# ProjectZKM/Ziren

Measured on AMD Instinct MI355X. Metric: shard-proofs/sec, higher is better.
Workload: dtype u32

## Files before the change

### include/zkm_hip.h

```cpp
#ifndef ZKM_HIP_H
#define ZKM_HIP_H

#include <stddef.h>
#include <stdint.h>

#ifdef __cplusplus
extern "C" {
#endif

#define ZKM_DIGEST_ELEMS 8
#define ZKM_EXT_DEGREE 4
#define ZKM_PERM_WIDTH 16
#define ZKM_KOALABEAR_P 0x7f000001u

typedef struct zkm_ctx zkm_ctx;
typedef struct zkm_matrix zkm_matrix;
typedef struct zkm_pcs_data zkm_pcs_data;
typedef struct zkm_pk zkm_pk;
typedef struct zkm_main_data zkm_main_data;

typedef struct {
  uint32_t log_blowup;
  uint32_t num_queries;
  uint32_t proof_of_work_bits;
// ... 44 lines not shown
const char* zkm_last_error(void);
const char* zkm_build_info(void);

int zkm_ctx_create(int device, zkm_ctx** out);
void zkm_ctx_destroy(zkm_ctx* ctx);
int zkm_ctx_synchronize(zkm_ctx* ctx);
int zkm_ctx_trim(zkm_ctx* ctx);
int zkm_ctx_set_memory_limit(zkm_ctx* ctx, size_t bytes);
size_t zkm_ctx_memory_held(zkm_ctx* ctx);
int zkm_ctx_last_timings(zkm_ctx* ctx, const char** names, float* ms, int cap);
int zkm_ctx_kernel_timings(zkm_ctx* ctx, const char** names, float* ms, uint32_t* calls, double* bytes, int cap);
void zkm_ctx_set_kernel_timing(zkm_ctx* ctx, int mode);
void zkm_ctx_set_kernel_timing_only(zkm_ctx* ctx, const char* name);
void zkm_ctx_set_lde_overlap(zkm_ctx* ctx, int on);
void zkm_ctx_set_rows_up_front(zkm_ctx* ctx, int on);
void zkm_ctx_set_host_wait(zkm_ctx* ctx, int blocking);
int zkm_ctx_register_quotient_kernel(zkm_ctx* ctx, const uint32_t* program, uint32_t program_len,
                                     const void* code_object, size_t code_object_len);

int zkm_ctx_register_perm_kernel(zkm_ctx* ctx, const uint32_t* lookups, uint32_t lookups_len, uint32_t log_quotient_degree,
                                 const void* code_object, size_t code_object_len);

void* zkm_host_alloc(zkm_ctx* ctx, size_t bytes);
void zkm_host_free(zkm_ctx* ctx, void* p);
int zkm_matrix_upload(zkm_ctx* ctx, const uint32_t* host_row_major, size_t height, size_t width,
                      zkm_matrix** out);
int zkm_matrix_upload_async(zkm_ctx* ctx, const uint32_t* host_row_major, size_t height, size_t width,
                            zkm_matrix** out);
int zkm_matrix_wait(zkm_ctx* ctx, const zkm_matrix* m);
int zkm_events_upload_async(zkm_ctx* ctx, const void* host_events, size_t bytes, void** device_events_out);
// ... 332 lines not shown
```

### integration/zkm-hip/src/ffi.rs

```rust
#![allow(non_camel_case_types, non_snake_case, dead_code)]
use core::ffi::{c_char, c_int, c_void};

pub const ZKM_DIGEST_ELEMS: u32 = 8;
pub const ZKM_EXT_DEGREE: u32 = 4;
pub const ZKM_PERM_WIDTH: u32 = 16;
pub const ZKM_KOALABEAR_P: u32 = 0x7f000001;
pub const ZKM_KECCAK_SPONGE_WIDTH: u32 = 3531;
pub const ZKM_SHA_EXTEND_WIDTH: u32 = 176;
pub const ZKM_SHA_COMPRESS_WIDTH: u32 = 262;
pub const ZKM_ED_ADD_WIDTH: u32 = 1861;
pub const ZKM_ED_DECOMPRESS_WIDTH: u32 = 1566;
pub const ZKM_GLOBAL_WIDTH: u32 = 99;

#[repr(C)] pub struct ZkmCtx { _private: [u8; 0] }
#[repr(C)] pub struct ZkmMatrix { _private: [u8; 0] }
#[repr(C)] pub struct ZkmPcsData { _private: [u8; 0] }
#[repr(C)] pub struct ZkmPk { _private: [u8; 0] }
#[repr(C)] pub struct ZkmMainData { _private: [u8; 0] }
#[repr(C)] pub struct ZkmByteLookups { _private: [u8; 0] }

#[repr(C)]
#[derive(Clone, Copy, Debug)]
pub struct ZkmFriConfig {
    pub log_blowup: u32,
// ... 412 lines not shown
extern "C" {
    pub fn zkm_last_error() -> *const c_char;
    pub fn zkm_build_info() -> *const c_char;
    pub fn zkm_ctx_create(device: c_int, out: *mut *mut ZkmCtx) -> c_int;
    pub fn zkm_ctx_destroy(ctx: *mut ZkmCtx);
    pub fn zkm_ctx_synchronize(ctx: *mut ZkmCtx) -> c_int;
    pub fn zkm_ctx_trim(ctx: *mut ZkmCtx) -> c_int;
    pub fn zkm_ctx_set_memory_limit(ctx: *mut ZkmCtx, bytes: usize) -> c_int;
    pub fn zkm_ctx_memory_held(ctx: *mut ZkmCtx) -> usize;
    pub fn zkm_ctx_last_timings(ctx: *mut ZkmCtx, names: *mut *const c_char, ms: *mut f32, cap: c_int) -> c_int;
    pub fn zkm_ctx_kernel_timings(ctx: *mut ZkmCtx, names: *mut *const c_char, ms: *mut f32, calls: *mut u32, bytes: *mut f64, cap: c_int) -> c_int;
    pub fn zkm_ctx_set_kernel_timing(ctx: *mut ZkmCtx, mode: c_int);
    pub fn zkm_ctx_set_kernel_timing_only(ctx: *mut ZkmCtx, name: *const c_char);
    pub fn zkm_ctx_set_lde_overlap(ctx: *mut ZkmCtx, on: c_int);
    pub fn zkm_ctx_set_rows_up_front(ctx: *mut ZkmCtx, on: c_int);
    pub fn zkm_ctx_set_host_wait(ctx: *mut ZkmCtx, blocking: c_int);
    pub fn zkm_ctx_register_quotient_kernel(ctx: *mut ZkmCtx, program: *const u32, program_len: u32, code_object: *const c_void, code_object_len: usize) -> c_int;
    pub fn zkm_ctx_register_perm_kernel(ctx: *mut ZkmCtx, lookups: *const u32, lookups_len: u32, log_quotient_degree: u32, code_object: *const c_void, code_object_len: usize) -> c_int;
    pub fn zkm_host_alloc(ctx: *mut ZkmCtx, bytes: usize) -> *mut c_void;
    pub fn zkm_host_free(ctx: *mut ZkmCtx, p: *mut c_void);
    pub fn zkm_matrix_upload(ctx: *mut ZkmCtx, host_row_major: *const u32, height: usize, width: usize, out: *mut *mut ZkmMatrix) -> c_int;
    pub fn zkm_matrix_upload_async(ctx: *mut ZkmCtx, host_row_major: *const u32, height: usize, width: usize, out: *mut *mut ZkmMatrix) -> c_int;
    pub fn zkm_matrix_wait(ctx: *mut ZkmCtx, m: *const ZkmMatrix) -> c_int;
    pub fn zkm_events_upload_async(ctx: *mut ZkmCtx, host_events: *const c_void, bytes: usize, device_events_out: *mut *mut c_void) -> c_int;
    pub fn zkm_events_free(ctx: *mut ZkmCtx, device_events: *mut c_void);
    pub fn zkm_matrix_download(ctx: *mut ZkmCtx, m: *const ZkmMatrix, host_row_major: *mut u32) -> c_int;
    pub fn zkm_matrix_height(m: *const ZkmMatrix) -> usize;
    pub fn zkm_matrix_width(m: *const ZkmMatrix) -> usize;
    pub fn zkm_matrix_free(ctx: *mut ZkmCtx, m: *mut ZkmMatrix);
    pub fn zkm_pcs_commit(ctx: *mut ZkmCtx, n_mats: usize, mats: *const *const ZkmMatrix, domain_shifts: *const u32, log_blowup: u32, root_out: *mut u32, out: *mut *mut ZkmPcsData) -> c_int;
// ... 84 lines not shown
```

### ziren_amd/csrc/host_ctx.hpp

```cpp
#pragma once
static thread_local std::string g_err;

#define HIP_CHECK(expr)                                                                          \
  do {                                                                                           \
    hipError_t _e = (expr);                                                                      \
    if (_e != hipSuccess)                                                                        \
      throw std::runtime_error(std::string(#expr) + ": " + hipGetErrorString(_e) + " (" + __FILE__ + ":" + \
                               std::to_string(__LINE__) + ")");                                  \
  } while (0)
#define LAUNCH_CHECK() HIP_CHECK(hipGetLastError())
#define KLAUNCH(ctx, name, bytes, kernel, grid, block, lds, ...)                                        \
  do {                                                                                                   \
    (ctx)->flush_staged();                                                                               \
    if ((ctx)->kbegin(name, (double)(bytes))) {                                                          \
       \
      hipExtLaunchKernelGGL(kernel, grid, block, lds, (ctx)->cur, (ctx)->krecs.back().start,             \
                            (ctx)->krecs.back().stop, 0, __VA_ARGS__);                                   \
    } else {                                                                                             \
      hipLaunchKernelGGL(kernel, grid, block, lds, (ctx)->cur, __VA_ARGS__);                             \
    }                                                                                                    \
    LAUNCH_CHECK();                                                                                      \
  } while (0)

static inline int log2_strict(size_t n) {
// ... 96 lines not shown
  std::mutex mu;
  std::multimap<size_t, void*> free_list;
  std::map<void*, size_t> live;
  std::map<int, uint32_t*> tw_fwd, tw_inv;
  std::vector<std::pair<std::string, hipEvent_t>> marks;
  std::vector<hipEvent_t> event_pool;
  std::vector<std::string> timing_names;
  std::vector<float> timing_ms;
  struct KRec { const char* name; double bytes; hipEvent_t start, stop; };
  struct KStat { double ms = 0, bytes = 0; uint32_t calls = 0; };
  std::vector<KRec> krecs;
  std::map<std::string, KStat> kstats;
  int kernel_timing = 2;
  bool lde_overlap = !(getenv("ZKM_LDE_OVERLAP") && atoi(getenv("ZKM_LDE_OVERLAP")) == 0);
  bool rows_up_front = !(getenv("ZKM_ROWS_UP_FRONT") && atoi(getenv("ZKM_ROWS_UP_FRONT")) == 0);
  bool root_poll = !(getenv("ZKM_ROOT_POLL") && atoi(getenv("ZKM_ROOT_POLL")) == 0);
  int root_spin_before_yield = getenv("ZKM_ROOT_SPIN") ? atoi(getenv("ZKM_ROOT_SPIN")) : 4096;
  int root_sleep_ns = getenv("ZKM_ROOT_SLEEP_NS") ? atoi(getenv("ZKM_ROOT_SLEEP_NS")) : 0;
  bool host_wait_blocking = getenv("ZKM_HOST_WAIT") && !strcmp(getenv("ZKM_HOST_WAIT"), "blocking");
  int wait_sleep_ns = getenv("ZKM_WAIT_SLEEP_NS") ? atoi(getenv("ZKM_WAIT_SLEEP_NS")) : 20000;
  struct TimerSlack {
    long saved = -1;
    void tighten() {
      if (saved >= 0) return;
      saved = prctl(PR_GET_TIMERSLACK, 0, 0, 0, 0);
      if (saved >= 0) prctl(PR_SET_TIMERSLACK, 1000UL, 0, 0, 0);
    }
    ~TimerSlack() { if (saved >= 0) prctl(PR_SET_TIMERSLACK, (unsigned long)saved, 0, 0, 0); }
  };
  static void sleep_ns(long ns, TimerSlack& slack) {
// ... 363 lines not shown
```

### ziren_amd/csrc/host_open.hpp

```cpp
#pragma once
static E4 host_pow2k(E4 a, int k) { return kb::epow2k(a, k); }

struct Writer {
  uint32_t* dst;
  size_t cap, n = 0;
  Writer(uint32_t* d, size_t c) : dst(d), cap(d ? c : 0) {}
  void u(uint32_t v) { if (n < cap) dst[n] = v; n++; }
  void words(const uint32_t* p, size_t cnt) {
    if (n < cap) memcpy(dst + n, p, std::min(cnt, cap - n) * 4);
    n += cnt;
  }
  void ext(const E4& e) { words(e.c, 4); }
  size_t size() const { return n; }
};

struct RoundMat {
  const uint32_t* evals; size_t n; size_t width; uint32_t shift;
  const zkm_matrix* lde;
  int n_points;
  std::vector<E4> y[2];
  size_t col0 = 0;
};
struct Round { const zkm_pcs_data* data; std::vector<RoundMat> mats; };

static const uint32_t SEPTIC_X[7] = {637514027, 1595065213, 1998064738, 72333738, 1211544370, 822986770, 1518535784};
static const uint32_t SEPTIC_Y[7] = {1604177449, 90440090, 259343427, 140470264, 1162099742, 941559812, 1064053343};

struct ChipMeta {
  const zkm_chip_desc* desc;
  int log_n;
  size_t n;
  int n_lookups, n_sends, perm_ext_w, max_values;
};

static ChipMeta chip_meta(const zkm_chip_desc* d, size_t n, size_t n_public_values) {
  ChipMeta m;
  m.desc = d; m.n = n; m.log_n = log2_strict(n);
  m.n_lookups = m.n_sends = m.max_values = 0;
  const std::string who = std::string(" (chip ") + (d->name ? d->name : "?") + ")";
  if (d->log_quotient_degree > 3) throw std::runtime_error("log_quotient_degree > 3 unsupported" + who);
  if (d->lookups_len) {
    const uint32_t* w = d->lookups;
    const size_t len = d->lookups_len;
    size_t pos = 0;
    auto need = [&](size_t k) { if (pos + k > len) throw std::runtime_error("lookup blob truncated" + who); };
    need(2);
    uint32_t ns = w[pos++], nr = w[pos++];
    if ((uint64_t)ns + nr > 4096) throw std::runtime_error("too many lookups" + who);
// ... 15 lines not shown
          if ((cw >> 31) ? col >= d->main_width : col >= d->prep_width) throw std::runtime_error("lookup column out of range" + who);
          if (weight >= kb::P) throw std::runtime_error("lookup weight not a field element" + who);
        }
      }
    }
    if (pos != len) throw std::runtime_error("lookup blob length mismatch" + who);
  }
  int batch = 1 << d->log_quotient_degree;
  m.perm_ext_w = m.n_lookups ? (m.n_lookups + batch - 1) / batch + 1 : 0;
  if (d->program_len) {
    if (d->program_len < 4 || d->program_len != 4 + 2 * (size_t)d->program[0]) throw std::runtime_error("program blob length mismatch" + who);
    if (d->program[2] != d->num_constraints) throw std::runtime_error("program constraint count mismatch" + who);
    const uint32_t ne = std::max<uint32_t>(d->program[1], 1), nb = std::max<uint32_t>(d->program[3], 1);
    if (ne > 256 || nb > 256) throw std::runtime_error("program register count out of range" + who);
    size_t asserts = 0;
    for (uint32_t k = 0; k < d->program[0]; k++) {
      uint32_t w0 = d->program[4 + 2 * k], imm = d->program[5 + 2 * k];
      uint32_t op = w0 & 0xff, dst = (w0 >> 8) & 0xff, ra = (w0 >> 16) & 0xff, rb = w0 >> 24;
      bool ok = true;
      switch (op) {
        case ZKM_OP_LD_MAIN: ok = dst < nb && ra < 2 && imm < d->main_width; break;
        case ZKM_OP_LD_PREP: ok = dst < nb && ra < 2 && imm < d->prep_width; break;
        case ZKM_OP_LD_PERM: ok = dst < ne && ra < 2 && imm < (uint32_t)m.perm_ext_w; break;
        case ZKM_OP_LD_CONST: ok = dst < nb && imm < kb::P; break;
        case ZKM_OP_LD_PV: ok = dst < nb && imm < n_public_values; break;
        case ZKM_OP_LD_CHALLENGE: ok = dst < ne && imm < 2; break;
        case ZKM_OP_LD_LOCAL_SUM: ok = dst < ne; break;
        case ZKM_OP_LD_GLOBAL_SUM: ok = dst < nb && imm < 14; break;
        case ZKM_OP_LD_IS_FIRST: case ZKM_OP_LD_IS_LAST: case ZKM_OP_LD_IS_TRANS: ok = dst < nb; break;
        case ZKM_OP_ADD_B: case ZKM_OP_SUB_B: case ZKM_OP_MUL_B: ok = dst < nb && ra < nb && rb < nb; break;
        case ZKM_OP_NEG_B: ok = dst < nb && ra < nb; break;
        case ZKM_OP_ADD_E: case ZKM_OP_SUB_E: case ZKM_OP_MUL_E: ok = dst < ne && ra < ne && rb < ne; break;
        case ZKM_OP_NEG_E: ok = dst < ne && ra < ne; break;
        case ZKM_OP_ADD_EB: case ZKM_OP_SUB_EB: case ZKM_OP_MUL_EB: ok = dst < ne && ra < ne && rb < nb; break;
        case ZKM_OP_ASSERT_B: ok = ra < nb; asserts++; break;
        case ZKM_OP_ASSERT_E: ok = ra < ne; asserts++; break;
        default: ok = false;
      }
      if (!ok) throw std::runtime_error("invalid instruction " + std::to_string(k) + " in constraint program" + who);
    }
    if (asserts != d->num_constraints) throw std::runtime_error("program asserts do not match num_constraints" + who);
  } else if (d->num_constraints) {
    throw std::runtime_error("num_constraints > 0 but no program" + who);
  }
  return m;
}

template <typename Alloc>
static void launch_permutation_trace(zkm_ctx* ctx, const ChipMeta& c, const uint32_t* d_blob, const uint32_t* trace, const uint32_t* prep, const E4& alpha,
                                     const E4* d_beta_powers, zkm_matrix& pt, Alloc&& salloc, std::vector<stark::ScanJob>& scans) {
  const double pbytes = 4.0 * c.n * (c.desc->main_width + c.desc->prep_width + pt.w);
  auto fit = c.desc->lookups_len ? ctx->perm_fns.find(perm_key(c.desc->lookups, c.desc->lookups_len, c.desc->log_quotient_degree)) : ctx->perm_fns.end();
  if (fit != ctx->perm_fns.end()) {
    stark::PermArgs a;
    a.main = trace; a.prep = prep; a.n = c.n; a.alpha = alpha; a.beta_pows = d_beta_powers; a.perm = pt.d;
    size_t arg_size = sizeof(a);
// ... 156 lines not shown
  for (size_t i = 0; i < nc; i++) {
    for (int e = 0; e < 4; e++) local_sums[i].c[e] = h_sums[18 * i + e];
    if (chips[i].desc->commit_scope_global) {
      for (int k = 0; k < 14; k++) global_sums[i][k] = h_sums[18 * i + 4 + k];
    } else {
      for (int k = 0; k < 7; k++) { global_sums[i][k] = kb::to_monty(SEPTIC_X[k]); global_sums[i][7 + k] = kb::to_monty(SEPTIC_Y[k]); }
    }
  }
  chal::observe_slice(ch, perm_data->root, 8);
  for (size_t i = 0; i < nc; i++) {
    chal::observe_ext(ch, local_sums[i]);
    chal::observe_slice(ch, global_sums[i].data(), 14);
  }
  }

  void quotient_phase() {
  E4 alpha = chal::sample_ext(ch);
  std::vector<std::function<void()>> launches;
  for (size_t i = 0; i < nc; i++) {
    const ChipMeta& c = chips[i];
    const zkm_chip_desc* d = c.desc;
    int lqd = d->log_quotient_degree;
    int lq = c.log_n + lqd;
    size_t Q = (size_t)1 << lq;
    size_t nchunks = (size_t)1 << lqd;
    uint32_t* qbuf = ctx->alloc_n<uint32_t>(Q * 4);
    scratch.push_back(qbuf);
    size_t C = d->num_constraints;
    std::vector<E4> ap(std::max<size_t>(C, 1));
    E4 p = kb::eone();
    for (size_t k = 0; k < C; k++) { ap[C - 1 - k] = p; p = kb::emul(p, alpha); }
    E4* d_ap = (E4*)ctx->upload_staged(ap.data(), ap.size() * sizeof(E4), &scratch);
    uint32_t consts[32] = {0};
    for (int k = 0; k < 14; k++) consts[k] = global_sums[i][k];
    uint32_t w_q = kb::two_adic_generator(lq);
    uint32_t s_pow_n = kb::pow(kb::GEN, (uint64_t)c.n);
    uint32_t wr = kb::two_adic_generator(lqd), wp = kb::ONE;
    for (size_t k = 0; k < nchunks; k++) {
      consts[16 + k] = kb::sub(kb::mul(s_pow_n, wp), kb::ONE);
      consts[24 + k] = kb::inv(consts[16 + k]);
      wp = kb::mul(wp, wr);
    }
// ... 11 lines not shown
    a.log_n = c.log_n; a.lqd = lqd;
    a.alpha_pows = d_ap; a.public_values = d_pv;
    a.perm_alpha = perm_ch[0]; a.perm_beta = perm_ch[1];
    a.local_sum = local_sums[i];
    a.consts = d_consts;
    a.w_q = w_q; a.g_inv = kb::inv(kb::two_adic_generator(c.log_n));
    a.out = qbuf;
    a.selectors = ctx->selectors(c.log_n, lqd, w_q, a.g_inv, d_consts);
    a.n_base_regs = d->program_len ? std::max<uint32_t>(d->program[3], 1) : 1;
    size_t per_thread = (size_t)a.n_regs * 16 + (size_t)a.n_base_regs * 4;
    int bd = 256;
    while (per_thread * bd > 64 * 1024 && bd > 64) bd >>= 1;
    size_t lds = per_thread * bd;
    if (lds > 152 * 1024) throw std::runtime_error(std::string("constraint program of chip ") + d->name + " needs too many registers");
    double qbytes = 4.0 * Q * (d->main_width + d->prep_width + 4.0 * c.perm_ext_w) + 16.0 * Q;
    auto fit = d->program_len ? ctx->quotient_fns.find(fnv1a(d->program, d->program_len)) : ctx->quotient_fns.end();
    const bool special = fit != ctx->quotient_fns.end();
    const std::vector<hipFunction_t>* fns = special ? &fit->second : nullptr;
    hipFunction_t uni_fn = nullptr;
    a.uniforms = nullptr;
    if (special) {
      auto uit = ctx->quotient_uniform_fns.find(fit->first);
      if (uit != ctx->quotient_uniform_fns.end()) {
        uni_fn = uit->second;
        a.uniforms = ctx->alloc_n<uint32_t>(stark::QUOTIENT_UNIFORM_WORDS);
        scratch.push_back(a.uniforms);
      }
    }
    launches.push_back([this, a, fns, uni_fn, Q, bd, lds, qbytes]() mutable {
      if (fns) {
        size_t arg_size = sizeof(a);
// ... 426 lines not shown
```

### ziren_amd/csrc/host_pcs.hpp

```cpp
#pragma once
struct LdeJob {
  const uint32_t* in; size_t n, w; uint32_t lde_shift; uint32_t* out;
  uint32_t* cflag = nullptr;
  bool uniform = false;
};

static void lde_batch_chunk(zkm_ctx* ctx, const std::vector<LdeJob>& jobs, int bl) {
  std::vector<size_t> order(jobs.size());
  std::iota(order.begin(), order.end(), 0);
  std::stable_sort(order.begin(), order.end(), [&](size_t a, size_t b) { return jobs[a].n > jobs[b].n; });
  std::vector<lde::Batch> hb(1);
  lde::Batch& b = hb[0];
  memset(&b, 0, sizeof b);
  b.log_blowup = bl;
  const size_t cosets = (size_t)1 << bl;
  size_t tmp1_words = 0, tmp2_words = 0;
  for (size_t oi : order) if (jobs[oi].n > ((size_t)1 << lde::LOG_ROW_MAX)) { tmp1_words += jobs[oi].n * jobs[oi].w; tmp2_words += (jobs[oi].n * jobs[oi].w) << bl; }
  uint32_t* tmp1 = tmp1_words ? ctx->alloc_n<uint32_t>(tmp1_words) : nullptr;
  uint32_t* tmp2 = tmp2_words ? ctx->alloc_n<uint32_t>(tmp2_words) : nullptr;
  size_t t1 = 0, t2 = 0;
  size_t big_cols = 0, fc = 0;
  for (size_t oi : order) if (jobs[oi].n > ((size_t)1 << lde::LOG_ROW_MAX) && !jobs[oi].cflag) big_cols += jobs[oi].w;
  uint32_t* cflags = big_cols ? ctx->alloc_n<uint32_t>(2 * big_cols) : nullptr;
  if (cflags) HIP_CHECK(hipMemsetAsync(cflags, 0, 2 * big_cols * sizeof(uint32_t), ctx->cur));
// ... 13 lines not shown
    g.n_inv = kb::inv(kb::to_monty((uint32_t)(n % kb::P)));
    g.twb_inv = lb > 0 ? ctx->twiddles(lb, true) : nullptr;
    g.twb_fwd = lb > 0 ? ctx->twiddles(lb, false) : nullptr;
    if (la) {
      g.twa_inv = ctx->twiddles_ct(la, true);
      g.twa_fwd = ctx->twiddles_ct(la, false);
      auto pw = ctx->pow_tables(k);
      g.pw_lo = pw.first; g.pw_hi = pw.second;
      g.tw_rows = ctx->row_twiddles(k);
    }
    uint32_t cols = 0;
    for (; p < order.size() && jobs[order[p]].n == n; p++) {
      const LdeJob& j = jobs[order[p]];
      lde::Mat& m = b.m[nm++];
      m.in = j.in; m.out = j.out; m.col0 = cols; m.w = (uint32_t)j.w; m.shift = j.lde_shift; m.uniform = j.uniform ? 1u : 0u;
      if (la) {
        m.tmp1 = tmp1 + t1; t1 += n * j.w;
        m.tmp2 = tmp2 + t2; t2 += (n * j.w) << bl;
        if (j.cflag) m.cflag = j.cflag;
        else { m.cflag = cflags + fc; fc += 2 * j.w; }
        auto ct = ctx->coset_tables(k, bl, j.lde_shift);
        m.twf = ct.twf; m.cs = ct.cs;
      }
      cols += (uint32_t)j.w;
    }
    g.n_cols = cols;
    g.n_mats = nm - g.first_mat;
    const double cells = (double)n * cols;
    if (la) {
      const size_t per_col = ((size_t)1 << lb) >> g.logT;
      blk[lde::K_COLS_INV] += (uint32_t)(per_col * cols);
      blk[lde::K_ROWS_BIG] += (uint32_t)(((size_t)1 << la) * cols);
      blk[lde::K_COLS_FWD] += (uint32_t)(per_col * cols * cosets);
      lds_cols = std::max(lds_cols, ((size_t)1 << la) * (((size_t)1 << g.logT) + 1) * 4);
      bytes_inv += 8.0 * cells; bytes_rows += 4.0 * cells * (1 + cosets); bytes_fwd += 8.0 * cells * cosets;
      for (int mi = (int)g.first_mat; mi < nm; mi++) if (b.m[mi].uniform) bytes_inv -= 8.0 * (double)n * b.m[mi].w;
    } else {
      blk[lde::K_ROWS_SMALL] += cols;
      const size_t B = (size_t)1 << lb;
      lds_small = std::max(lds_small, (2 * (B + (B >> 5)) + 64 + (B > 64 ? (B >> 6) : 1)) * 4);
      bytes_small += 4.0 * cells * (1 + cosets);
    }
    for (int q = 0; q < 4; q++) g.blk_end[q] = blk[q];
    b.n_groups++;
  }
  const lde::Batch* d = (const lde::Batch*)ctx->upload_staged(&b, sizeof b);
  if (blk[lde::K_COLS_INV]) {
    constexpr size_t B = (size_t)1 << lde::LOG_ROW_MAX;
    const size_t big_lds = (B + (B >> 5)) * 4;
    KLAUNCH(ctx, "lde_cols_inverse", bytes_inv, lde::lde_cols<false>, dim3(blk[lde::K_COLS_INV]), dim3(lde::THREADS), lds_cols, d);
    KLAUNCH(ctx, "lde_rows", bytes_rows, lde::lde_rows_big, dim3(blk[lde::K_ROWS_BIG]), dim3(lde::THREADS), big_lds, d);
// ... 324 lines not shown
```

### ziren_amd/csrc/lde.cuh

```cuda
#pragma once
#include "kb31.cuh"
#include "gptr.cuh"

namespace lde {

constexpr int LOG_ROW_MAX = 13;
constexpr int THREADS = 512;

template <bool PAD>
__device__ __forceinline__ uint32_t phys(uint32_t i) { return PAD ? i + (i >> 5) : i; }

template <bool DIF, int R, bool LAZY = false>
__device__ __forceinline__ void butterflies(uint32_t (&x)[1 << R], uint32_t n, uint32_t s0, uint32_t lo, uint32_t logm2,
                                            const uint32_t* __restrict__ tw) {
  static_assert(!(DIF && LAZY), "the lazy form exists for the DIT butterfly only");
#pragma unroll
  for (int qq = 0; qq < R; qq++) {
    const uint32_t q = DIF ? qq : R - 1 - qq;
    const uint32_t s = s0 + q;
    const uint32_t half = 1u << (R - 1 - q);
    const uint32_t tbase = (n - (n >> s)) + lo;
#pragma unroll
    for (uint32_t j0 = 0; j0 < (1u << R); j0++) {
      if (j0 & half) continue;
// ... 128 lines not shown
}

constexpr int MAX_GROUPS = 24, MAX_MATS = 64;
enum { K_COLS_INV = 0, K_ROWS_BIG = 1, K_COLS_FWD = 2, K_ROWS_SMALL = 3 };

struct Mat {
  const uint32_t* in;
  uint32_t* out;
  uint32_t* tmp1;
  uint32_t* tmp2;
  const uint32_t* twf;
  const uint32_t* cs;
  uint32_t col0, w;
  uint32_t shift;
  uint32_t uniform;
  uint32_t* cflag;
};
struct Group {
  int la, lb, logT, pad;
  uint32_t n_cols, first_mat, n_mats, pad2;
  uint32_t blk_end[4];
  const uint32_t *twb_fwd, *twb_inv;
  const uint32_t *twa_fwd, *twa_inv;
  const uint32_t *pw_lo, *pw_hi;
  const uint32_t* tw_rows;
  uint32_t w_N, n_inv, pad3[2];
};
struct Batch {
  int n_groups, log_blowup;
  Group g[MAX_GROUPS];
// ... 16 lines not shown
template <bool FORWARD>
__global__ __launch_bounds__(THREADS) void lde_cols(const Batch* __restrict__ d) {
  extern __shared__ uint32_t lds[];
  uint32_t local;
  const Group& g = find_group(d, FORWARD ? K_COLS_FWD : K_COLS_INV, local);
  const int la = g.la, lb = g.lb, logT = g.logT, log_blowup = d->log_blowup;
  const int A = 1 << la, T = 1 << logT, TP = T + 1;
  const size_t B = (size_t)1 << lb, n = (size_t)A << lb;
  const uint32_t xb = local & ((1u << (lb - logT)) - 1);
  const uint32_t rest = local >> (lb - logT);
  const uint32_t col = FORWARD ? rest % g.n_cols : rest;
  const int z = FORWARD ? (int)(rest / g.n_cols) : 0;
  const Mat& m = find_mat(d, g, col);
  const size_t c = col - m.col0;
  const size_t t0 = (size_t)xb << logT;
  const uint32_t* src = (FORWARD ? m.tmp2 + (size_t)z * n * m.w : m.in) + c * n + t0;
  const uint32_t* __restrict__ tw = FORWARD ? g.twa_fwd : g.twa_inv;
  const int logTq = logT - 2;
  const int quads = (A << logT) >> 2;
  if (!FORWARD && m.uniform) {
    if (xb == 0 && threadIdx.x == 0) gp::store(m.cflag + 2 * c + 1, gp::load(m.in + c * n));
    return;
  }
  if (FORWARD && gp::load(m.cflag + 2 * c) == 0) {
    const uint32_t v0 = gp::load(m.cflag + 2 * c + 1);
    const uint32_t v = kb::umin32(v0, v0 - kb::P);
    uint32_t* dst = m.out + c * (n << log_blowup) + (size_t)kb::bitrev(z, log_blowup) * n;
    if (la < 2) {
      for (int u = threadIdx.x; u < (A << logT); u += blockDim.x)
        gp::store(dst + (size_t)kb::bitrev((uint32_t)(t0 + (u >> la)), lb) * A + (u & (A - 1)), v);
      return;
// ... 17 lines not shown
#pragma unroll
    for (int k = 0; k < 4; k++) {
      int u = u0 + k * blockDim.x;
      if (u < quads) {
        uint32_t* dd = lds + (u >> logTq) * TP + ((u & ((1 << logTq) - 1)) << 2);
        dd[0] = v[k].x; dd[1] = v[k].y; dd[2] = v[k].z; dd[3] = v[k].w;
        if (!FORWARD) differs |= (v[k].x ^ first_word) | (v[k].y ^ first_word) | (v[k].z ^ first_word) | (v[k].w ^ first_word);
      }
    }
  }
  if (!FORWARD) {
    if (__any(differs != 0) && (threadIdx.x & 63) == 0) gp::store(m.cflag + 2 * c, 1u);
    if (xb == 0 && threadIdx.x == 0) gp::store(m.cflag + 2 * c + 1, first_word);
  }
  __syncthreads();
  const bool fused_last = la >= 2 && (la & 3) == 1;
  lds_ntt_ct<false>(lds, la, logT, TP, tw, fused_last);
  const uint32_t* __restrict__ tw_last = tw + ((1u << (la - 1)) - 1);
  if (!FORWARD) {
    uint32_t* dst = m.tmp1 + c * n + t0;
    if (fused_last) {
      for (int u0 = threadIdx.x; u0 < (quads >> 1); u0 += blockDim.x) {
        const int rp = u0 >> logTq, qd = (u0 & ((1 << logTq) - 1)) << 2;
        const uint32_t* sp = lds + (2 * rp) * TP + qd;
        uint32_t x[4] = {sp[0], sp[1], sp[2], sp[3]}, y[4] = {sp[TP], sp[TP + 1], sp[TP + 2], sp[TP + 3]};
        const uint32_t w = gp::load(tw_last + rp);
#pragma unroll
        for (int k = 0; k < 4; k++) last_stage_ct(x[k], y[k], w);
        gp::store(reinterpret_cast<uint4*>(dst + (size_t)(2 * rp) * B + qd), make_uint4(x[0], x[1], x[2], x[3]));
        gp::store(reinterpret_cast<uint4*>(dst + (size_t)(2 * rp + 1) * B + qd), make_uint4(y[0], y[1], y[2], y[3]));
// ... 98 lines not shown
  __syncthreads();
  ntt_pass_ct<4, true>(work, LB, 4, twr);
  ntt_pass_ct<4, true>(work, LB, 8, twr);
  uint32_t keep[16];
#pragma unroll
  for (uint32_t k = 0; k < 8; k++) {
    const uint32_t gg = tid + (k << 9);
    const int32_t a = (int32_t)work[phys<true>(2 * gg)], b = (int32_t)work[phys<true>(2 * gg + 1)];
    const uint32_t w = gp::load(twr + (1u << 12) - 1 + gg);
    const int64_t ar = kb::mad_i64_i32_uniform(a, kb::ONE, 0);
    keep[2 * k] = (uint32_t)kb::monty_reduce_signed(kb::mad_i64_i32(b, (int32_t)w, ar));
    keep[2 * k + 1] = (uint32_t)kb::monty_reduce_signed(kb::mad_i64_i32(-b, (int32_t)w, ar));
  }
  const uint32_t st0 = pw((k1 * tid) & nmask), st_step = pw((k1 << 9) & nmask);
  const uint32_t ncosets = 1u << d->log_blowup;
  for (uint32_t j = 0; j < ncosets; j++) {
    const uint32_t* __restrict__ tw_fwd = m.twf + (size_t)j * B;
    const uint32_t t_first = gp::load(tw_fwd + B - 2);
    const uint32_t cj = gp::load(m.cs + (j << la) + k1);
    __syncthreads();
    uint32_t lt = tid;
    asm volatile("" : "+v"(lt));
#pragma unroll
    for (uint32_t k = 0; k < 8; k++) {
      const uint32_t gg = lt + (k << 9);
      const int64_t ar = kb::mad_i64_i32_uniform((int32_t)keep[2 * k], kb::ONE, 0);
      work[phys<true>(2 * gg)] = (uint32_t)kb::monty_reduce_signed(kb::mad_i64_i32_uniform((int32_t)keep[2 * k + 1], t_first, ar));
      work[phys<true>(2 * gg + 1)] = (uint32_t)kb::monty_reduce_signed(kb::mad_i64_i32_uniform((int32_t)keep[2 * k + 1], 0u - t_first, ar));
    }
    __syncthreads();
    ntt_pass<false, 4, true, true>(work, LB, 0, 1, 8, tw_fwd, lt);
// ... 68 lines not shown
```

### ziren_amd/csrc/zkm_hip.hip

```cpp
#include "../../include/zkm_hip.h"

#include <hip/hip_runtime.h>
#include <hip/hip_ext.h>

#include <algorithm>
#include <array>
#include <atomic>
#include <chrono>
#include <cstdlib>
#include <cstdio>
#include <cstring>
#include <functional>
#include <map>
#include <mutex>
#include <numeric>
#include <stdexcept>
#include <string>
#include <unordered_map>
#include <exception>
#include <vector>

#include <sched.h>
#include <time.h>
#include <sys/prctl.h>
// ... 208 lines not shown
}

int zkm_ctx_kernel_timings(zkm_ctx* ctx, const char** names, float* ms, uint32_t* calls, double* bytes, int cap) {
  int i = 0;
  for (auto& kv : ctx->kstats) {
    if (i < cap) { names[i] = kv.first.c_str(); ms[i] = (float)kv.second.ms; calls[i] = kv.second.calls; bytes[i] = kv.second.bytes; }
    i++;
  }
  return i;
}
void zkm_ctx_set_kernel_timing(zkm_ctx* ctx, int mode) { ctx->kernel_timing = mode; }
void zkm_ctx_set_kernel_timing_only(zkm_ctx* ctx, const char* name) { ctx->timing_only = name ? name : ""; ctx->kernel_timing = 3; }
void zkm_ctx_set_host_wait(zkm_ctx* ctx, int blocking) { std::lock_guard<std::mutex> lk(ctx->mu); ctx->host_wait_blocking = blocking != 0; }
void zkm_ctx_set_lde_overlap(zkm_ctx* ctx, int on) { std::lock_guard<std::mutex> lk(ctx->mu); ctx->lde_overlap = on != 0; }
void zkm_ctx_set_rows_up_front(zkm_ctx* ctx, int on) { std::lock_guard<std::mutex> lk(ctx->mu); ctx->rows_up_front = on != 0; }

int zkm_ctx_register_quotient_kernel(zkm_ctx* ctx, const uint32_t* program, uint32_t program_len, const void* code_object,
                                     size_t code_object_len) {
  API_BEGIN
  std::lock_guard<std::mutex> lk(ctx->mu);
  HIP_CHECK(hipSetDevice(ctx->device));
  CallScope call_scope(ctx);
  if (!program_len || !code_object_len) throw std::runtime_error("empty program or code object");
  std::vector<std::pair<const char*, size_t>> parts;
  std::vector<std::vector<char>> copies;
  const char* bytes = (const char*)code_object;
  if (code_object_len >= 16 && memcmp(bytes, "ZKMQPART", 8) == 0) {
    uint32_t count;
    memcpy(&count, bytes + 8, 4);
    size_t at = 16 + 8 * (size_t)count;
// ... 536 lines not shown
```

### ziren_amd/lib.py

```python
import ctypes as C
import importlib.util
import os

from . import abi

HERE = os.path.dirname(os.path.abspath(__file__))
LIB_PATH = os.environ.get("ZKM_HIP_LIB") or os.path.join(HERE, "libzkm_hip.so")
_LIB = None

EXPORTS = [
    "zkm_last_error", "zkm_build_info", "zkm_ctx_create", "zkm_ctx_destroy", "zkm_ctx_synchronize", "zkm_ctx_trim", "zkm_ctx_set_memory_limit", "zkm_ctx_memory_held", "zkm_ctx_last_timings", "zkm_ctx_kernel_timings", "zkm_ctx_set_kernel_timing", "zkm_ctx_set_kernel_timing_only", "zkm_ctx_set_lde_overlap", "zkm_ctx_set_rows_up_front", "zkm_ctx_set_host_wait", "zkm_ctx_register_quotient_kernel", "zkm_ctx_register_perm_kernel",
    "zkm_host_alloc", "zkm_host_free", "zkm_matrix_upload", "zkm_matrix_upload_async", "zkm_matrix_wait", "zkm_events_upload_async", "zkm_events_free", "zkm_matrix_download", "zkm_matrix_height", "zkm_matrix_width", "zkm_matrix_free",
    "zkm_pcs_commit", "zkm_pcs_data_free", "zkm_pcs_data_get_lde", "zkm_pcs_open_batch",
    "zkm_pk_setup", "zkm_pk_commitment", "zkm_pk_observe_into", "zkm_pk_free",
    "zkm_commit", "zkm_main_data_free", "zkm_open", "zkm_prove_shard",
    "zkm_tracegen_alu_width", "zkm_byte_lookups_create", "zkm_byte_lookups_free", "zkm_tracegen_alu", "zkm_tracegen_jump_width", "zkm_tracegen_jump", "zkm_tracegen_branch_width", "zkm_tracegen_branch", "zkm_tracegen_mov_cond_width", "zkm_tracegen_mov_cond", "zkm_tracegen_mul_width", "zkm_tracegen_mul", "zkm_tracegen_divrem_width", "zkm_tracegen_divrem", "zkm_tracegen_cpu_width", "zkm_tracegen_cpu", "zkm_tracegen_cpu_and_program", "zkm_tracegen_program", "zkm_tracegen_program_mults", "zkm_tracegen_memory_local", "zkm_tracegen_global", "zkm_tracegen_misc_instrs_width", "zkm_tracegen_misc_instrs", "zkm_tracegen_syscall_instrs_width", "zkm_tracegen_syscall_instrs", "zkm_tracegen_syscall", "zkm_tracegen_memory_global", "zkm_tracegen_poseidon2_permute", "zkm_tracegen_keccak_sponge", "zkm_tracegen_sha_extend", "zkm_tracegen_sha_compress", "zkm_tracegen_ed_add", "zkm_tracegen_ed_decompress", "zkm_tracegen_weierstrass_add", "zkm_tracegen_weierstrass_double", "zkm_tracegen_weierstrass_decompress", "zkm_tracegen_uint256_mul", "zkm_tracegen_u256x2048_mul", "zkm_tracegen_boolean_circuit_garble", "zkm_tracegen_sys_linux", "zkm_tracegen_fp_op", "zkm_tracegen_fp2_addsub", "zkm_tracegen_fp2_mul", "zkm_tracegen_poseidon2_wide", "zkm_tracegen_poseidon2_skinny", "zkm_tracegen_exp_reverse_bits", "zkm_tracegen_memory_instrs_width", "zkm_tracegen_memory_instrs", "zkm_tracegen_flat", "zkm_tracegen_byte_table", "zkm_tracegen_byte_mults", "zkm_tracegen_shard",
    "zkm_poseidon2_permute_batch", "zkm_poseidon2_permute_batch_int", "zkm_coset_lde_batch", "zkm_permutation_trace",
    "zkm_challenger_init", "zkm_challenger_observe", "zkm_challenger_sample", "zkm_challenger_sample_bits",
    "zkm_host_poseidon2_permute", "zkm_host_poseidon2_permute_f64", "zkm_host_poseidon2_f64_sponge", "zkm_host_poseidon2_f64_compress_inject", "zkm_host_poseidon2_f64_audit",
    "zkm_host_ext_mul", "zkm_host_ext_inv", "zkm_host_field_mul", "zkm_host_field_inv", "zkm_host_reduce96_bounded", "zkm_host_two_adic_generator",
]


class ZkmError(RuntimeError):
    pass


def _preload_hip_runtime():
    try:
        spec = importlib.util.find_spec("torch")
    except (ImportError, ValueError):
        spec = None
    if spec is None or not spec.submodule_search_locations:
        return
    path = os.path.join(list(spec.submodule_search_locations)[0], "lib", "libamdhip64.so")
# ... 36 lines not shown
    L.zkm_tracegen_branch_width.restype = C.c_size_t
    L.zkm_tracegen_mul_width.restype = C.c_size_t
    L.zkm_tracegen_divrem_width.restype = C.c_size_t
    L.zkm_tracegen_cpu_width.restype = C.c_size_t
    L.zkm_tracegen_misc_instrs_width.restype = C.c_size_t
    L.zkm_tracegen_syscall_instrs_width.restype = C.c_size_t
    L.zkm_tracegen_memory_instrs_width.restype = C.c_size_t
    L.zkm_challenger_sample.restype = C.c_uint32
    L.zkm_challenger_sample_bits.restype = C.c_uint32
    L.zkm_host_field_mul.restype = C.c_uint32
    L.zkm_host_field_inv.restype = C.c_uint32
    if hasattr(L, "zkm_host_reduce96_bounded"):
        L.zkm_host_reduce96_bounded.restype = C.c_uint32
        L.zkm_host_reduce96_bounded.argtypes = [C.c_uint32, C.c_uint64]
    L.zkm_host_two_adic_generator.restype = C.c_uint32
    for name in ("zkm_ctx_destroy", "zkm_host_free", "zkm_events_free", "zkm_byte_lookups_free", "zkm_ctx_set_kernel_timing", "zkm_ctx_set_kernel_timing_only", "zkm_ctx_set_lde_overlap", "zkm_ctx_set_rows_up_front", "zkm_ctx_set_host_wait", "zkm_matrix_free", "zkm_pcs_data_free", "zkm_pk_free", "zkm_main_data_free",
                 "zkm_challenger_init", "zkm_challenger_observe", "zkm_host_poseidon2_permute", "zkm_host_poseidon2_permute_f64", "zkm_host_poseidon2_f64_sponge",
                 "zkm_host_poseidon2_f64_compress_inject", "zkm_host_poseidon2_f64_audit", "zkm_host_ext_mul", "zkm_host_ext_inv"):
        if hasattr(L, name) or "ZKM_HIP_LIB" not in os.environ:
            getattr(L, name).restype = None
    _LIB = L
    return L


def build_info():
    L = load()
    if not hasattr(L, "zkm_build_info"):
        return {}
    return dict(kv.split("=", 1) for kv in L.zkm_build_info().decode().split(";") if "=" in kv)


# ... 15 lines not shown
```

Baseline: 9.445.

## Skip quotient for provably-zero chips and copy LDE coset equal to trace domain

Adds a selector taint analysis of each constraint program. For chips with uniform rows, no preprocessed columns, selector-linear constraints and a zero local sum, the quotient is known to be zero, so the buffer is memset instead of running the quotient kernel. Separately, when one LDE coset shift equals one (the original domain), the forward NTT for that coset is replaced by a bit-reversed copy of the input. Both paths are on by default behind env toggles. The zero-quotient shortcut rests on a soundness argument that could be wrong for some programs.

```diff
diff --git a/include/zkm_hip.h b/include/zkm_hip.h
--- a/include/zkm_hip.h
+++ b/include/zkm_hip.h
@@ -82,6 +82,9 @@
 void zkm_ctx_set_kernel_timing_only(zkm_ctx* ctx, const char* name);
 void zkm_ctx_set_lde_overlap(zkm_ctx* ctx, int on);
 void zkm_ctx_set_rows_up_front(zkm_ctx* ctx, int on);
+void zkm_ctx_set_quotient_skip_zero(zkm_ctx* ctx, int on);
+void zkm_ctx_set_lde_copy_coset(zkm_ctx* ctx, int on);
+int zkm_host_program_selectors_linear(const uint32_t* program, uint32_t program_len);
 void zkm_ctx_set_host_wait(zkm_ctx* ctx, int blocking);
 int zkm_ctx_register_quotient_kernel(zkm_ctx* ctx, const uint32_t* program, uint32_t program_len,
                                      const void* code_object, size_t code_object_len);
diff --git a/integration/zkm-hip/src/ffi.rs b/integration/zkm-hip/src/ffi.rs
--- a/integration/zkm-hip/src/ffi.rs
+++ b/integration/zkm-hip/src/ffi.rs
@@ -450,6 +450,9 @@
     pub fn zkm_ctx_set_kernel_timing_only(ctx: *mut ZkmCtx, name: *const c_char);
     pub fn zkm_ctx_set_lde_overlap(ctx: *mut ZkmCtx, on: c_int);
     pub fn zkm_ctx_set_rows_up_front(ctx: *mut ZkmCtx, on: c_int);
+    pub fn zkm_ctx_set_quotient_skip_zero(ctx: *mut ZkmCtx, on: c_int);
+    pub fn zkm_ctx_set_lde_copy_coset(ctx: *mut ZkmCtx, on: c_int);
+    pub fn zkm_host_program_selectors_linear(program: *const u32, program_len: u32) -> c_int;
     pub fn zkm_ctx_set_host_wait(ctx: *mut ZkmCtx, blocking: c_int);
     pub fn zkm_ctx_register_quotient_kernel(ctx: *mut ZkmCtx, program: *const u32, program_len: u32, code_object: *const c_void, code_object_len: usize) -> c_int;
     pub fn zkm_ctx_register_perm_kernel(ctx: *mut ZkmCtx, lookups: *const u32, lookups_len: u32, log_quotient_degree: u32, code_object: *const c_void, code_object_len: usize) -> c_int;
diff --git a/ziren_amd/csrc/host_ctx.hpp b/ziren_amd/csrc/host_ctx.hpp
--- a/ziren_amd/csrc/host_ctx.hpp
+++ b/ziren_amd/csrc/host_ctx.hpp
@@ -134,6 +134,8 @@
   int kernel_timing = 2;
   bool lde_overlap = !(getenv("ZKM_LDE_OVERLAP") && atoi(getenv("ZKM_LDE_OVERLAP")) == 0);
   bool rows_up_front = !(getenv("ZKM_ROWS_UP_FRONT") && atoi(getenv("ZKM_ROWS_UP_FRONT")) == 0);
+  bool quotient_skip_zero = !(getenv("ZKM_QUOTIENT_SKIP_ZERO") && atoi(getenv("ZKM_QUOTIENT_SKIP_ZERO")) == 0);
+  bool lde_copy_coset = !(getenv("ZKM_LDE_COPY_COSET") && atoi(getenv("ZKM_LDE_COPY_COSET")) == 0);
   bool root_poll = !(getenv("ZKM_ROOT_POLL") && atoi(getenv("ZKM_ROOT_POLL")) == 0);
   int root_spin_before_yield = getenv("ZKM_ROOT_SPIN") ? atoi(getenv("ZKM_ROOT_SPIN")) : 4096;
   int root_sleep_ns = getenv("ZKM_ROOT_SLEEP_NS") ? atoi(getenv("ZKM_ROOT_SLEEP_NS")) : 0;
diff --git a/ziren_amd/csrc/host_open.hpp b/ziren_amd/csrc/host_open.hpp
--- a/ziren_amd/csrc/host_open.hpp
+++ b/ziren_amd/csrc/host_open.hpp
@@ -31,7 +31,32 @@
   int log_n;
   size_t n;
   int n_lookups, n_sends, perm_ext_w, max_values;
+  uint64_t program_key = 0;
+  bool selectors_linear = true;
 };
+
+struct SelectorTaint {
+  std::bitset<256> base, ext;
+  bool linear = true;
+  void step(uint32_t op, uint32_t dst, uint32_t ra, uint32_t rb) {
+    switch (op) {
+      case ZKM_OP_LD_IS_FIRST: case ZKM_OP_LD_IS_LAST: case ZKM_OP_LD_IS_TRANS: base[dst] = true; break;
+      case ZKM_OP_LD_MAIN: case ZKM_OP_LD_PREP: case ZKM_OP_LD_CONST: case ZKM_OP_LD_PV: case ZKM_OP_LD_GLOBAL_SUM: base[dst] = false; break;
+      case ZKM_OP_LD_PERM: case ZKM_OP_LD_CHALLENGE: case ZKM_OP_LD_LOCAL_SUM: ext[dst] = false; break;
+      case ZKM_OP_MUL_B: linear &= !(base[ra] && base[rb]); [[fallthrough]];
+      case ZKM_OP_ADD_B: case ZKM_OP_SUB_B: base[dst] = base[ra] || base[rb]; break;
+      case ZKM_OP_NEG_B: base[dst] = base[ra]; break;
+      case ZKM_OP_MUL_E: linear &= !(ext[ra] && ext[rb]); [[fallthrough]];
+      case ZKM_OP_ADD_E: case ZKM_OP_SUB_E: ext[dst] = ext[ra] || ext[rb]; break;
+      case ZKM_OP_NEG_E: ext[dst] = ext[ra]; break;
+      case ZKM_OP_MUL_EB: linear &= !(ext[ra] && base[rb]); [[fallthrough]];
+      case ZKM_OP_ADD_EB: case ZKM_OP_SUB_EB: ext[dst] = ext[ra] || base[rb]; break;
+      default: break;
+    }
+  }
+};
+static std::mutex g_selectors_mu;
+static std::map<uint64_t, bool> g_selectors_linear;
 
 static ChipMeta chip_meta(const zkm_chip_desc* d, size_t n, size_t n_public_values) {
   ChipMeta m;
@@ -77,9 +102,19 @@
     const uint32_t ne = std::max<uint32_t>(d->program[1], 1), nb = std::max<uint32_t>(d->program[3], 1);
     if (ne > 256 || nb > 256) throw std::runtime_error("program register count out of range" + who);
     size_t asserts = 0;
+    m.program_key = fnv1a(d->program, d->program_len);
+    bool known;
+    {
+      std::lock_guard<std::mutex> lk(g_selectors_mu);
+      auto it = g_selectors_linear.find(m.program_key);
+      known = it != g_selectors_linear.end();
+      if (known) m.selectors_linear = it->second;
+    }
+    SelectorTaint taint;
     for (uint32_t k = 0; k < d->program[0]; k++) {
       uint32_t w0 = d->program[4 + 2 * k], imm = d->program[5 + 2 * k];
       uint32_t op = w0 & 0xff, dst = (w0 >> 8) & 0xff, ra = (w0 >> 16) & 0xff, rb = w0 >> 24;
+      if (!known) taint.step(op, dst, ra, rb);
       bool ok = true;
       switch (op) {
         case ZKM_OP_LD_MAIN: ok = dst < nb && ra < 2 && imm < d->main_width; break;
@@ -103,6 +138,11 @@
       if (!ok) throw std::runtime_error("invalid instruction " + std::to_string(k) + " in constraint program" + who);
     }
     if (asserts != d->num_constraints) throw std::runtime_error("program asserts do not match num_constraints" + who);
+    if (!known) {
+      m.selectors_linear = taint.linear;
+      std::lock_guard<std::mutex> lk(g_selectors_mu);
+      g_selectors_linear[m.program_key] = taint.linear;
+    }
   } else if (d->num_constraints) {
     throw std::runtime_error("num_constraints > 0 but no program" + who);
   }
@@ -289,6 +329,14 @@
   }
   }
 
+  bool quotient_known_zero(size_t i) const {
+    const ChipMeta& c = chips[i];
+    if (!ctx->quotient_skip_zero || !md->traces[i].uniform_rows || c.desc->prep_index >= 0 || c.desc->prep_width || c.n < 4 || !c.selectors_linear)
+      return false;
+    for (int e = 0; e < 4; e++) if (local_sums[i].c[e] != 0) return false;
+    return true;
+  }
+
   void quotient_phase() {
   E4 alpha = chal::sample_ext(ch);
   std::vector<std::function<void()>> launches;
@@ -301,6 +349,19 @@
     size_t nchunks = (size_t)1 << lqd;
     uint32_t* qbuf = ctx->alloc_n<uint32_t>(Q * 4);
     scratch.push_back(qbuf);
+    if (quotient_known_zero(i)) {
+      HIP_CHECK(hipMemsetAsync(qbuf, 0, Q * 4 * sizeof(uint32_t), st));
+      launches.push_back([] {});
+      uint32_t wq = kb::two_adic_generator(lq), wqp = kb::ONE;
+      for (size_t k = 0; k < nchunks; k++) {
+        zkm_matrix m; m.h = c.n; m.w = 4; m.d = qbuf + k * 4 * c.n; m.owned = (k == 0);
+        m.uniform_rows = true;
+        qchunks.push_back(m);
+        qshifts.push_back(kb::mul(kb::GEN, wqp));
+        wqp = kb::mul(wqp, wq);
+      }
+      continue;
+    }
     size_t C = d->num_constraints;
     std::vector<E4> ap(std::max<size_t>(C, 1));
     E4 p = kb::eone();
@@ -342,7 +403,7 @@
     size_t lds = per_thread * bd;
     if (lds > 152 * 1024) throw std::runtime_error(std::string("constraint program of chip ") + d->name + " needs too many registers");
     double qbytes = 4.0 * Q * (d->main_width + d->prep_width + 4.0 * c.perm_ext_w) + 16.0 * Q;
-    auto fit = d->program_len ? ctx->quotient_fns.find(fnv1a(d->program, d->program_len)) : ctx->quotient_fns.end();
+    auto fit = d->program_len ? ctx->quotient_fns.find(c.program_key) : ctx->quotient_fns.end();
     const bool special = fit != ctx->quotient_fns.end();
     const std::vector<hipFunction_t>* fns = special ? &fit->second : nullptr;
     hipFunction_t uni_fn = nullptr;
diff --git a/ziren_amd/csrc/host_pcs.hpp b/ziren_amd/csrc/host_pcs.hpp
--- a/ziren_amd/csrc/host_pcs.hpp
+++ b/ziren_amd/csrc/host_pcs.hpp
@@ -51,6 +51,12 @@
       const LdeJob& j = jobs[order[p]];
       lde::Mat& m = b.m[nm++];
       m.in = j.in; m.out = j.out; m.col0 = cols; m.w = (uint32_t)j.w; m.shift = j.lde_shift; m.uniform = j.uniform ? 1u : 0u;
+      m.zcopy = -1;
+      if (la && ctx->lde_copy_coset) {
+        uint32_t s = j.lde_shift % kb::P;
+        for (size_t z = 0; z < cosets; z++, s = kb::mul(s, g.w_N))
+          if (s == kb::ONE) { m.zcopy = (int32_t)z; break; }
+      }
       if (la) {
         m.tmp1 = tmp1 + t1; t1 += n * j.w;
         m.tmp2 = tmp2 + t2; t2 += (n * j.w) << bl;
@@ -71,7 +77,10 @@
       blk[lde::K_COLS_FWD] += (uint32_t)(per_col * cols * cosets);
       lds_cols = std::max(lds_cols, ((size_t)1 << la) * (((size_t)1 << g.logT) + 1) * 4);
       bytes_inv += 8.0 * cells; bytes_rows += 4.0 * cells * (1 + cosets); bytes_fwd += 8.0 * cells * cosets;
-      for (int mi = (int)g.first_mat; mi < nm; mi++) if (b.m[mi].uniform) bytes_inv -= 8.0 * (double)n * b.m[mi].w;
+      for (int mi = (int)g.first_mat; mi < nm; mi++) {
+        if (b.m[mi].uniform) bytes_inv -= 8.0 * (double)n * b.m[mi].w;
+        if (b.m[mi].zcopy >= 0) bytes_rows -= 4.0 * (double)n * b.m[mi].w;
+      }
     } else {
       blk[lde::K_ROWS_SMALL] += cols;
       const size_t B = (size_t)1 << lb;
diff --git a/ziren_amd/csrc/lde.cuh b/ziren_amd/csrc/lde.cuh
--- a/ziren_amd/csrc/lde.cuh
+++ b/ziren_amd/csrc/lde.cuh
@@ -166,6 +166,8 @@
   uint32_t col0, w;
   uint32_t shift;
   uint32_t uniform;
+  int32_t zcopy;
+  uint32_t pad;
   uint32_t* cflag;
 };
 struct Group {
@@ -212,7 +214,8 @@
   const Mat& m = find_mat(d, g, col);
   const size_t c = col - m.col0;
   const size_t t0 = (size_t)xb << logT;
-  const uint32_t* src = (FORWARD ? m.tmp2 + (size_t)z * n * m.w : m.in) + c * n + t0;
+  const bool copy = FORWARD && z == m.zcopy;
+  const uint32_t* src = (FORWARD && !copy ? m.tmp2 + (size_t)z * n * m.w : m.in) + c * n + t0;
   const uint32_t* __restrict__ tw = FORWARD ? g.twa_fwd : g.twa_inv;
   const int logTq = logT - 2;
   const int quads = (A << logT) >> 2;
@@ -260,6 +263,29 @@
     if (xb == 0 && threadIdx.x == 0) gp::store(m.cflag + 2 * c + 1, first_word);
   }
   __syncthreads();
+  if (FORWARD && copy) {
+    uint32_t* dst = m.out + c * (n << log_blowup) + (size_t)kb::bitrev(z, log_blowup) * n;
+    if (la < 2) {
+      for (int u = threadIdx.x; u < (A << logT); u += blockDim.x) {
+        const int t = u >> la, q = u & (A - 1);
+        const uint32_t v = lds[q * TP + t];
+        gp::store(dst + (size_t)kb::bitrev((uint32_t)(t0 + t), lb) * A + q, kb::umin32(v, v - kb::P));
+      }
+      return;
+    }
+    const int logAq = la - 2;
+    for (int u0 = threadIdx.x; u0 < quads; u0 += blockDim.x) {
+      const int t = u0 >> logAq, q = (u0 & ((1 << logAq) - 1)) << 2;
+      uint32_t x[4];
+#pragma unroll
+      for (int k = 0; k < 4; k++) {
+        const uint32_t v = lds[kb::bitrev((uint32_t)(q + k), la) * TP + t];
+        x[k] = kb::umin32(v, v - kb::P);
+      }
+      gp::store(reinterpret_cast<uint4*>(dst + (size_t)kb::bitrev((uint32_t)(t0 + t), lb) * A + q), make_uint4(x[0], x[1], x[2], x[3]));
+    }
+    return;
+  }
   const bool fused_last = la >= 2 && (la & 3) == 1;
   lds_ntt_ct<false>(lds, la, logT, TP, tw, fused_last);
   const uint32_t* __restrict__ tw_last = tw + ((1u << (la - 1)) - 1);
@@ -388,7 +414,9 @@
   }
   const uint32_t st0 = pw((k1 * tid) & nmask), st_step = pw((k1 << 9) & nmask);
   const uint32_t ncosets = 1u << d->log_blowup;
+  const int32_t zcopy = m.zcopy;
   for (uint32_t j = 0; j < ncosets; j++) {
+    if ((int32_t)j == zcopy) continue;
     const uint32_t* __restrict__ tw_fwd = m.twf + (size_t)j * B;
     const uint32_t t_first = gp::load(tw_fwd + B - 2);
     const uint32_t cj = gp::load(m.cs + (j << la) + k1);
diff --git a/ziren_amd/csrc/zkm_hip.hip b/ziren_amd/csrc/zkm_hip.hip
--- a/ziren_amd/csrc/zkm_hip.hip
+++ b/ziren_amd/csrc/zkm_hip.hip
@@ -6,6 +6,7 @@
 #include <algorithm>
 #include <array>
 #include <atomic>
+#include <bitset>
 #include <chrono>
 #include <cstdlib>
 #include <cstdio>
@@ -246,6 +247,18 @@
 void zkm_ctx_set_host_wait(zkm_ctx* ctx, int blocking) { std::lock_guard<std::mutex> lk(ctx->mu); ctx->host_wait_blocking = blocking != 0; }
 void zkm_ctx_set_lde_overlap(zkm_ctx* ctx, int on) { std::lock_guard<std::mutex> lk(ctx->mu); ctx->lde_overlap = on != 0; }
 void zkm_ctx_set_rows_up_front(zkm_ctx* ctx, int on) { std::lock_guard<std::mutex> lk(ctx->mu); ctx->rows_up_front = on != 0; }
+void zkm_ctx_set_quotient_skip_zero(zkm_ctx* ctx, int on) { std::lock_guard<std::mutex> lk(ctx->mu); ctx->quotient_skip_zero = on != 0; }
+void zkm_ctx_set_lde_copy_coset(zkm_ctx* ctx, int on) { std::lock_guard<std::mutex> lk(ctx->mu); ctx->lde_copy_coset = on != 0; }
+
+int zkm_host_program_selectors_linear(const uint32_t* program, uint32_t program_len) {
+  if (!program || program_len < 4 || program_len != 4 + 2 * (size_t)program[0]) { g_err = "zkm_host_program_selectors_linear: program blob length mismatch"; return -1; }
+  SelectorTaint taint;
+  for (uint32_t k = 0; k < program[0]; k++) {
+    const uint32_t w0 = program[4 + 2 * k];
+    taint.step(w0 & 0xff, (w0 >> 8) & 0xff, (w0 >> 16) & 0xff, w0 >> 24);
+  }
+  return taint.linear ? 1 : 0;
+}
 
 int zkm_ctx_register_quotient_kernel(zkm_ctx* ctx, const uint32_t* program, uint32_t program_len, const void* code_object,
                                      size_t code_object_len) {
diff --git a/ziren_amd/lib.py b/ziren_amd/lib.py
--- a/ziren_amd/lib.py
+++ b/ziren_amd/lib.py
@@ -9,7 +9,7 @@
 _LIB = None
 
 EXPORTS = [
-    "zkm_last_error", "zkm_build_info", "zkm_ctx_create", "zkm_ctx_destroy", "zkm_ctx_synchronize", "zkm_ctx_trim", "zkm_ctx_set_memory_limit", "zkm_ctx_memory_held", "zkm_ctx_last_timings", "zkm_ctx_kernel_timings", "zkm_ctx_set_kernel_timing", "zkm_ctx_set_kernel_timing_only", "zkm_ctx_set_lde_overlap", "zkm_ctx_set_rows_up_front", "zkm_ctx_set_host_wait", "zkm_ctx_register_quotient_kernel", "zkm_ctx_register_perm_kernel",
+    "zkm_last_error", "zkm_build_info", "zkm_ctx_create", "zkm_ctx_destroy", "zkm_ctx_synchronize", "zkm_ctx_trim", "zkm_ctx_set_memory_limit", "zkm_ctx_memory_held", "zkm_ctx_last_timings", "zkm_ctx_kernel_timings", "zkm_ctx_set_kernel_timing", "zkm_ctx_set_kernel_timing_only", "zkm_ctx_set_lde_overlap", "zkm_ctx_set_rows_up_front", "zkm_ctx_set_quotient_skip_zero", "zkm_ctx_set_lde_copy_coset", "zkm_ctx_set_host_wait", "zkm_ctx_register_quotient_kernel", "zkm_ctx_register_perm_kernel",
     "zkm_host_alloc", "zkm_host_free", "zkm_matrix_upload", "zkm_matrix_upload_async", "zkm_matrix_wait", "zkm_events_upload_async", "zkm_events_free", "zkm_matrix_download", "zkm_matrix_height", "zkm_matrix_width", "zkm_matrix_free",
     "zkm_pcs_commit", "zkm_pcs_data_free", "zkm_pcs_data_get_lde", "zkm_pcs_open_batch",
     "zkm_pk_setup", "zkm_pk_commitment", "zkm_pk_observe_into", "zkm_pk_free",
@@ -18,7 +18,7 @@
     "zkm_poseidon2_permute_batch", "zkm_poseidon2_permute_batch_int", "zkm_coset_lde_batch", "zkm_permutation_trace",
     "zkm_challenger_init", "zkm_challenger_observe", "zkm_challenger_sample", "zkm_challenger_sample_bits",
     "zkm_host_poseidon2_permute", "zkm_host_poseidon2_permute_f64", "zkm_host_poseidon2_f64_sponge", "zkm_host_poseidon2_f64_compress_inject", "zkm_host_poseidon2_f64_audit",
-    "zkm_host_ext_mul", "zkm_host_ext_inv", "zkm_host_field_mul", "zkm_host_field_inv", "zkm_host_reduce96_bounded", "zkm_host_two_adic_generator",
+    "zkm_host_ext_mul", "zkm_host_ext_inv", "zkm_host_field_mul", "zkm_host_field_inv", "zkm_host_reduce96_bounded", "zkm_host_two_adic_generator", "zkm_host_program_selectors_linear",
 ]
 
 
@@ -85,7 +85,7 @@
         L.zkm_host_reduce96_bounded.restype = C.c_uint32
         L.zkm_host_reduce96_bounded.argtypes = [C.c_uint32, C.c_uint64]
     L.zkm_host_two_adic_generator.restype = C.c_uint32
-    for name in ("zkm_ctx_destroy", "zkm_host_free", "zkm_events_free", "zkm_byte_lookups_free", "zkm_ctx_set_kernel_timing", "zkm_ctx_set_kernel_timing_only", "zkm_ctx_set_lde_overlap", "zkm_ctx_set_rows_up_front", "zkm_ctx_set_host_wait", "zkm_matrix_free", "zkm_pcs_data_free", "zkm_pk_free", "zkm_main_data_free",
+    for name in ("zkm_ctx_destroy", "zkm_host_free", "zkm_events_free", "zkm_byte_lookups_free", "zkm_ctx_set_kernel_timing", "zkm_ctx_set_kernel_timing_only", "zkm_ctx_set_lde_overlap", "zkm_ctx_set_rows_up_front", "zkm_ctx_set_quotient_skip_zero", "zkm_ctx_set_lde_copy_coset", "zkm_ctx_set_host_wait", "zkm_matrix_free", "zkm_pcs_data_free", "zkm_pk_free", "zkm_main_data_free",
                  "zkm_challenger_init", "zkm_challenger_observe", "zkm_host_poseidon2_permute", "zkm_host_poseidon2_permute_f64", "zkm_host_poseidon2_f64_sponge",
                  "zkm_host_poseidon2_f64_compress_inject", "zkm_host_poseidon2_f64_audit", "zkm_host_ext_mul", "zkm_host_ext_inv"):
         if hasattr(L, name) or "ZKM_HIP_LIB" not in os.environ:
```

New measurement: 23.90, median of 6. +153.0%, better.
